# ANRGUSC/DEFER

Measured on NVIDIA H100. Metric: inferences_per_sec, higher is better.
Workload: dtype bf16x3->f32

## Files before the change

defer_b200/csrc/conv_umma.cu:

```cuda
#include <cuda.h>
#include <string.h>

#include <type_traits>

#include <vector>

#include "common.cuh"
#include "conv_umma.cuh"

namespace defer {

static int env_int(const char* name, int dflt) {
  const char* v = getenv(name);
  return v ? atoi(v) : dflt;
}

namespace {

constexpr int BM = 128;
constexpr int BK = 64;
constexpr int CONS_THREADS = 256;
constexpr int NUM_THREADS = CONS_THREADS + 128;
constexpr int SMEM_CAP = 227 * 1024 - 256;
constexpr int CTL_BYTES = 256;
// ... 7 lines not shown
  int tile_n, tile_h, tile_w, tiles_h, tiles_w;
  int flat;
  int m_total;
  int kh, kw, sh, sw, pad_t, pad_l;
  int cblocks;
  int k_blocks;
  int splits;
  int cluster;
  uint32_t flags;
  const float* scale;
  const float* shift;
  const void* res;
  void* y;
  float* partial;
  unsigned int* counters;
  size_t plane_out;
};

struct alignas(128) MegaOp {
  CUtensorMap tmx[2];
  CUtensorMap tmw[2];
  KParams p;
  int m_tiles, n_tiles;
  const float* stem_x;
  int stem_h, stem_w, stem_cin, stem_kh, stem_kw, stem_sh, stem_sw, stem_pad_t, stem_pad_l, stem_K;
  int stem_win_rows, stem_win_cols;
  const uint8_t* stem_u8;
  float stem_shift[3];
  const float* scale2;
  const float* shift2;
  void* y2;
  int relu2;
  int store_first;
};

template <int NPLANES, int BN>
struct Smem {
  static constexpr int A_PLANE = BM * 128;
  static constexpr int B_PLANE = BN * 128;
  static constexpr int STAGE = NPLANES * (A_PLANE + B_PLANE);
  static constexpr int RED = BM * BN * 4;
  __host__ __device__ static constexpr int ring(int stages, bool red) {
    return (red && stages * STAGE < RED) ? RED : stages * STAGE;
  }
  __host__ __device__ static constexpr int total(int stages, bool red) {
    return ring(stages, red) + STG_BYTES + CTL_BYTES + 1024;
  }
  __host__ __device__ static constexpr int max_stages() {
    return (SMEM_CAP - STG_BYTES - CTL_BYTES - 1024) / STAGE > MAX_STAGES ? MAX_STAGES
                                                                          : (SMEM_CAP - STG_BYTES - CTL_BYTES - 1024) / STAGE;
  }
};
static_assert(Smem<2, 128>::max_stages() == 3 && Smem<2, 64>::max_stages() == 4, "BF16X2 ring depths");
static_assert(Smem<1, 64>::max_stages() == 8 && Smem<1, 128>::max_stages() == 6, "BF16 ring depths");

__device__ __forceinline__ uint32_t smem_u32(const void* p) { return (uint32_t)__cvta_generic_to_shared(p); }

__device__ __forceinline__ void mbar_init(uint32_t bar, uint32_t count) {
  asm volatile("mbarrier.init.shared::cta.b64 [%0], %1;" ::"r"(bar), "r"(count));
}
__device__ __forceinline__ void mbar_arrive_expect_tx(uint32_t bar, uint32_t bytes) {
  asm volatile("mbarrier.arrive.expect_tx.shared::cta.b64 _, [%0], %1;" ::"r"(bar), "r"(bytes) : "memory");
}
__device__ __forceinline__ void mbar_expect_tx(uint32_t bar, uint32_t bytes) {
  asm volatile("mbarrier.expect_tx.relaxed.cta.shared::cta.b64 [%0], %1;" ::"r"(bar), "r"(bytes) : "memory");
}
// ... 147 lines not shown
  int cout;
  bool relu;
  bool store_first;
  bool relu2;
  const float* scale2;
  const float* shift2;
  __nv_bfloat16* y2;
};

__device__ __forceinline__ EpiArgs epi_args(const MegaOp& op) {
  const KParams& p = op.p;
  EpiArgs e;
  e.scale = p.scale;
  e.shift = p.shift;
  e.res = reinterpret_cast<const __nv_bfloat16*>(p.res);
  e.y = reinterpret_cast<__nv_bfloat16*>(p.y);
  e.plane = p.plane_out;
  e.cout = p.cout;
  e.relu = (p.flags & DEFER_FLAG_RELU) != 0;
  e.store_first = op.store_first != 0;
  e.relu2 = op.relu2 != 0;
  e.scale2 = op.scale2;
  e.shift2 = op.shift2;
  e.y2 = reinterpret_cast<__nv_bfloat16*>(op.y2);
  return e;
}

__device__ __forceinline__ uint32_t stg_off(int r, int c) {
  return (uint32_t)(r * STG_COLS + (((c >> 2) ^ ((r & 7) << 1)) << 2) + (c & 3)) * 4u;
}
__device__ __forceinline__ void sts2(uint32_t addr, float a, float b) {
  asm volatile("st.shared.v2.f32 [%0], {%1, %2};" ::"r"(addr), "f"(a), "f"(b));
}
__device__ __forceinline__ float4 lds4(uint32_t addr) {
  float4 v;
  asm volatile("ld.shared.v4.f32 {%0, %1, %2, %3}, [%4];" : "=f"(v.x), "=f"(v.y), "=f"(v.z), "=f"(v.w) : "r"(addr));
  return v;
}
__device__ __forceinline__ void stg4(void* p, uint4 v) {
  asm volatile("st.global.v4.b32 [%0], {%1, %2, %3, %4};" ::"l"(p), "r"(v.x), "r"(v.y), "r"(v.z), "r"(v.w));
}

__device__ __forceinline__ float bf_lo(uint32_t w) { return __uint_as_float(w << 16); }
__device__ __forceinline__ float bf_hi(uint32_t w) { return __uint_as_float(w & 0xffff0000u); }

template <int NPLANES, int BN, bool AFF>
__device__ __forceinline__ void epi_tile(const KParams& p, const EpiArgs& e, uint32_t stg, const float (&acc)[BN / 2],
                                         uint32_t qmask, int c_base, int n0, int h0, int w0) {
  const int tid = threadIdx.x;
  const int lane = tid & 31;
  const int row0 = (tid >> 7) * 64 + ((tid >> 5) & 3) * 16 + (lane >> 2);
  const int col_l = 2 * (lane & 3);
  const int jg = tid & 7;
  const int rb = tid >> 3;
  const int ca = 2 * jg + ((jg >> 2) & 1), cb = ca ^ 1;
  const bool swap = (jg >> 2) & 1;
  size_t orow[4];
  uint32_t vmask = 0;
#pragma unroll
  for (int k = 0; k < 4; ++k) {
    bool v;
    size_t pix;
    row_to_pixel(p, rb + 32 * k, n0, h0, w0, v, pix);
    orow[k] = pix * (size_t)e.cout;
    vmask |= (uint32_t)v << k;
  }
#pragma unroll
  for (int P = 0; P < BN / STG_COLS; ++P) {
    const bool mine = (qmask >> (8 * P + jg)) & 1u;
    const int c = c_base + STG_COLS * P + 8 * jg;
    cons_bar_sync();
#pragma unroll
    for (int qq = 0; qq < 8; ++qq) {
      const int q = 8 * P + qq;
      if (!((qmask >> q) & 1u)) continue;
      sts2(stg + stg_off(row0, 8 * qq + col_l), acc[4 * q], acc[4 * q + 1]);
      sts2(stg + stg_off(row0 + 8, 8 * qq + col_l), acc[4 * q + 2], acc[4 * q + 3]);
    }
    uint4 rh[4], rl[4];
// ... 20 lines not shown
        sf[0] = a.x; sf[1] = a.y; sf[2] = a.z; sf[3] = a.w; sf[4] = b.x; sf[5] = b.y; sf[6] = b.z; sf[7] = b.w;
      }
    }
    cons_bar_sync();
    if (!mine) continue;

#pragma unroll
    for (int k = 0; k < 4; ++k) {
      if (!((vmask >> k) & 1u)) continue;
      const int r = rb + 32 * k;
      const float4 xa = lds4(stg + stg_off(r, 4 * ca));
      const float4 xb = lds4(stg + stg_off(r, 4 * cb));
      const float4 x0 = swap ? xb : xa, x1 = swap ? xa : xb;
      float v[8] = {x0.x, x0.y, x0.z, x0.w, x1.x, x1.y, x1.z, x1.w};
      const uint32_t hw[4] = {rh[k].x, rh[k].y, rh[k].z, rh[k].w};
      const uint32_t lw[4] = {rl[k].x, rl[k].y, rl[k].z, rl[k].w};
#pragma unroll
      for (int i = 0; i < 8; ++i) {
        v[i] = fmaf(v[i], sc[i], sf[i]);
        if (e.res) {
          v[i] += (i & 1) ? bf_hi(hw[i >> 1]) : bf_lo(hw[i >> 1]);
          if (NPLANES == 2) v[i] += (i & 1) ? bf_hi(lw[i >> 1]) : bf_lo(lw[i >> 1]);
        }
        if (e.relu) v[i] = fmaxf(v[i], 0.f);
      }
      uint4 hi, lo = make_uint4(0u, 0u, 0u, 0u);
      if (NPLANES == 2) {
        split_bf16x2(v[0], v[1], hi.x, lo.x);
        split_bf16x2(v[2], v[3], hi.y, lo.y);
        split_bf16x2(v[4], v[5], hi.z, lo.z);
        split_bf16x2(v[6], v[7], hi.w, lo.w);
      } else {
        hi = make_uint4(pack_bf16x2(v[0], v[1]), pack_bf16x2(v[2], v[3]), pack_bf16x2(v[4], v[5]), pack_bf16x2(v[6], v[7]));
      }
      const size_t o = orow[k] + c;
      if (!AFF || e.store_first) {
        stg4(e.y + o, hi);
        if (NPLANES == 2) stg4(e.y + e.plane + o, lo);
      }
      if constexpr (AFF) {
        float s2[8], t2[8];
        {
          const float4 a = __ldg(reinterpret_cast<const float4*>(e.scale2 + c));
          const float4 b = __ldg(reinterpret_cast<const float4*>(e.scale2 + c + 4));
          const float4 d = __ldg(reinterpret_cast<const float4*>(e.shift2 + c));
          const float4 f = __ldg(reinterpret_cast<const float4*>(e.shift2 + c + 4));
          s2[0] = a.x; s2[1] = a.y; s2[2] = a.z; s2[3] = a.w; s2[4] = b.x; s2[5] = b.y; s2[6] = b.z; s2[7] = b.w;
          t2[0] = d.x; t2[1] = d.y; t2[2] = d.z; t2[3] = d.w; t2[4] = f.x; t2[5] = f.y; t2[6] = f.z; t2[7] = f.w;
        }
        const uint32_t sh[4] = {hi.x, hi.y, hi.z, hi.w};
        const uint32_t sl[4] = {lo.x, lo.y, lo.z, lo.w};
        float u[8];
#pragma unroll
        for (int i = 0; i < 8; ++i) {
          u[i] = (i & 1) ? bf_hi(sh[i >> 1]) : bf_lo(sh[i >> 1]);
          if (NPLANES == 2) u[i] = u[i] + ((i & 1) ? bf_hi(sl[i >> 1]) : bf_lo(sl[i >> 1]));
          u[i] = fmaf(u[i], s2[i], t2[i]);
          if (e.relu2) u[i] = fmaxf(u[i], 0.f);
        }
        uint4 h2, l2;
        if (NPLANES == 2) {
          split_bf16x2(u[0], u[1], h2.x, l2.x);
          split_bf16x2(u[2], u[3], h2.y, l2.y);
          split_bf16x2(u[4], u[5], h2.z, l2.z);
          split_bf16x2(u[6], u[7], h2.w, l2.w);
          stg4(e.y2 + o, h2);
// ... 337 lines not shown
template <int NPLANES>
__device__ __forceinline__ void stem_build(const StemGeo& g, uint32_t win, uint32_t a_dst, int r, int row_base, int kb) {
  int k = kb * BK;
  int a = k / g.run, jj = k - a * g.run;
  uint32_t src = win + 4u * (uint32_t)(row_base + a * g.wcols + jj);
  const uint32_t wrap = 4u * (uint32_t)(g.wcols - g.run);
#pragma unroll 1
  for (int ch = 0; ch < 8; ++ch) {
    float v[8];
#pragma unroll
    for (int e = 0; e < 8; ++e) {
      v[e] = 0.f;
      if (k < g.K) asm volatile("ld.shared.f32 %0, [%1];" : "=f"(v[e]) : "r"(src));
      ++k;
      src += 4u;
      if (++jj == g.run) { jj = 0; src += wrap; }
    }
    const uint32_t off = (uint32_t)r * 128u + ((uint32_t)(ch ^ (r & 7)) << 4);
    uint32_t h[4], l[4];
#pragma unroll
    for (int q = 0; q < 4; ++q) {
      if (NPLANES == 2) split_bf16x2(v[2 * q], v[2 * q + 1], h[q], l[q]);
      else h[q] = pack_bf16x2(v[2 * q], v[2 * q + 1]);
    }
    asm volatile("st.shared.v4.b32 [%0], {%1, %2, %3, %4};" ::"r"(a_dst + off), "r"(h[0]), "r"(h[1]), "r"(h[2]), "r"(h[3])
                 : "memory");
    if (NPLANES == 2)
      asm volatile("st.shared.v4.b32 [%0], {%1, %2, %3, %4};" ::"r"(a_dst + Smem<NPLANES, 64>::A_PLANE + off), "r"(l[0]),
                   "r"(l[1]), "r"(l[2]), "r"(l[3])
                   : "memory");
  }
}

template <int NPLANES, int IN>
__device__ __forceinline__ void stem_body(const MegaOp* ops, int stages, int pdl) {
  using L = Smem<NPLANES, 64>;
  extern __shared__ uint8_t smem_raw[];
  uint8_t* smem = reinterpret_cast<uint8_t*>((reinterpret_cast<uintptr_t>(smem_raw) + 1023) & ~(uintptr_t)1023);
  const uint32_t ring = smem_u32(smem);
  const uint32_t stg = ring + stages * L::STAGE;
  const uint32_t win0 = stg + STG_BYTES;
  const uint32_t bar_base = win0 + 2 * STEM_WIN_BYTES;
  auto full_bar = [&](int s) { return bar_base + 8u * s; };
  auto empty_bar = [&](int s) { return bar_base + 8u * (stages + s); };

  const int tid = threadIdx.x;
  if (tid == 0) {
    for (int s = 0; s < stages; ++s) {
      mbar_init(full_bar(s), 1);
      mbar_init(empty_bar(s), CONS_THREADS / 32);
    }
    asm volatile("fence.mbarrier_init.release.cluster;" ::: "memory");
  }
  __syncthreads();
  if (pdl) {
    asm volatile("griddepcontrol.wait;" ::: "memory");
    asm volatile("griddepcontrol.launch_dependents;" ::: "memory");
  }

  const MegaOp& op = ops[0];
  const KParams& p = op.p;
  const int total = op.m_tiles * op.n_tiles;
  const int k_blocks = p.k_blocks;
  uint32_t it = 0;

  if (tid >= CONS_THREADS) {
// ... 11 lines not shown
    }
    int wb = 0;
    for (int t = blockIdx.x; t < total; t += gridDim.x, wb ^= 1) {
      const int t_next = t + (int)gridDim.x;
      if (t_next < total) {
        stem_tile_origin(p, t_next % op.m_tiles, n0, h0, w0);
        stem_fill_load<IN>(g, ptid, n0, h0, w0, raw);
      }
      prod_bar_sync();
      const uint32_t win = win0 + (uint32_t)wb * STEM_WIN_BYTES;
      const int c_base = (t / op.m_tiles) * 64;
      for (int kb = 0; kb < k_blocks; ++kb, ++it) {
        const int stage = (int)(it % (uint32_t)stages);
        mbar_wait(empty_bar(stage), ((it / (uint32_t)stages) & 1u) ^ 1u, 1);
        const uint32_t a_dst = ring + stage * L::STAGE;
        const uint32_t b_dst = a_dst + NPLANES * L::A_PLANE;
        if (ptid == 0) {
          mbar_expect_tx(full_bar(stage), NPLANES * (uint32_t)L::B_PLANE);
          tma_load_3d(b_dst, &op.tmw[0], full_bar(stage), kb * BK, c_base, 0);
          if (NPLANES == 2) tma_load_3d(b_dst + L::B_PLANE, &op.tmw[1], full_bar(stage), kb * BK, c_base, 0);
        }
        stem_build<NPLANES>(g, win, a_dst, ptid, row_base, kb);
        asm volatile("fence.proxy.async.shared::cta;" ::: "memory");
        prod_bar_sync();
        if (ptid == 0) mbar_arrive(full_bar(stage));
      }
      if (t_next < total) stem_fill_store<IN>(g, win0 + (uint32_t)(wb ^ 1) * STEM_WIN_BYTES, ptid, raw);
    }
    return;
  }

  const int wg = tid >> 7;
  const int lane = tid & 31;
  for (int t = blockIdx.x; t < total; t += gridDim.x) {
    float acc[32];
#pragma unroll
    for (int i = 0; i < 32; ++i) acc[i] = 0.f;
    int prev_stage = -1;
    for (int kb = 0; kb < k_blocks; ++kb, ++it) {
      const int stage = (int)(it % (uint32_t)stages);
      mbar_wait(full_bar(stage), (it / (uint32_t)stages) & 1u, 2);
      const uint32_t a_addr = ring + stage * L::STAGE + wg * (64 * 128);
      const uint32_t b_addr = ring + stage * L::STAGE + NPLANES * L::A_PLANE;
      wg_fence();
#pragma unroll
      for (int k = 0; k < BK / 16; ++k) {
        const uint64_t a_hi = make_sw128_desc(a_addr + k * 32);
        const uint64_t b_hi = make_sw128_desc(b_addr + k * 32);
        wgmma_bf16<64>(acc, a_hi, b_hi);
        if (NPLANES == 2) {
          wgmma_bf16<64>(acc, make_sw128_desc(a_addr + L::A_PLANE + k * 32), b_hi);
          wgmma_bf16<64>(acc, a_hi, make_sw128_desc(b_addr + L::B_PLANE + k * 32));
        }
      }
      wg_commit();
      wg_wait<1>();
      acc_fence(acc);
      if (prev_stage >= 0 && lane == 0) mbar_arrive(empty_bar(prev_stage));
      prev_stage = stage;
    }
    wg_wait<0>();
    acc_fence(acc);
    if (prev_stage >= 0 && lane == 0) mbar_arrive(empty_bar(prev_stage));
    int n0, h0, w0;
    stem_tile_origin(p, t % op.m_tiles, n0, h0, w0);
    epi_tile<NPLANES, 64, false>(p, epi_args(op), stg, acc, 0xffffu, (t / op.m_tiles) * 64, n0, h0, w0);
  }
}

template <int NPLANES>
__global__ void __launch_bounds__(NUM_THREADS, 1) conv_stem_kernel(const MegaOp* __restrict__ ops, int stages, int pdl) {
  stem_body<NPLANES, STEM_F32>(ops, stages, pdl);
}

template <int NPLANES>
__global__ void __launch_bounds__(NUM_THREADS, 1) conv_stem_u8_kernel(const MegaOp* __restrict__ ops, int stages, int pdl) {
  stem_body<NPLANES, STEM_U8_CAFFE>(ops, stages, pdl);
}

template <int NPLANES>
__global__ void __launch_bounds__(NUM_THREADS, 1) conv_stem_u8tf_kernel(const MegaOp* __restrict__ ops, int stages, int pdl) {
  stem_body<NPLANES, STEM_U8_TF>(ops, stages, pdl);
}

__global__ void __launch_bounds__(256) weight_transform_kernel(const float* __restrict__ w, __nv_bfloat16* __restrict__ out,
                                                               int taps, int cin, int cout, int nplanes) {
  size_t total = (size_t)taps * cin * cout;
  size_t i = (size_t)blockIdx.x * blockDim.x + threadIdx.x;
  if (i >= total) return;
  int ci = (int)(i % cin);
  size_t t2 = i / cin;
  int co = (int)(t2 % cout);
  int tap = (int)(t2 / cout);
  float v = w[((size_t)tap * cin + ci) * cout + co];
  __nv_bfloat16 hi = __float2bfloat16_rn(v);
  out[i] = hi;
  if (nplanes == 2) out[total + i] = __float2bfloat16_rn(v - __bfloat162float(hi));
}

// ... 441 lines not shown
bool umma_stem_fusable(int fmt, int cin, int ho, int wo, int cout, int kh, int kw, int sh, int sw, uint32_t flags) {
  if (fmt != FMT_BF16X2 && fmt != FMT_BF16) return false;
  if (cout != 64 || (flags & DEFER_FLAG_RESIDUAL) || kh * kw * cin > 256) return false;
  int tile_h, tile_w, win_rows, win_cols;
  stem_tile(ho, wo, kh, kw, sh, sw, cin, &tile_h, &tile_w, &win_rows, &win_cols);
  return (long long)win_rows * win_cols <= STEM_WIN_VALS;
}

int umma_mega_set_stem(void* host_op, const float* x, int h, int w, int cin, int kh, int kw, int sh, int sw, int pad_t,
                       int pad_l) {
  MegaOp* op = reinterpret_cast<MegaOp*>(host_op);
  KParams& p = op->p;
  op->stem_x = x;
  op->stem_h = h; op->stem_w = w; op->stem_cin = cin;
  op->stem_kh = kh; op->stem_kw = kw; op->stem_sh = sh; op->stem_sw = sw;
  op->stem_pad_t = pad_t; op->stem_pad_l = pad_l;
  op->stem_K = kh * kw * cin;
  stem_tile(p.ho, p.wo, kh, kw, sh, sw, cin, &p.tile_h, &p.tile_w, &op->stem_win_rows, &op->stem_win_cols);
  p.flat = 0;
  p.tile_n = 1;
  p.tiles_h = (p.ho + p.tile_h - 1) / p.tile_h;
  p.tiles_w = (p.wo + p.tile_w - 1) / p.tile_w;
  op->m_tiles = p.n * p.tiles_h * p.tiles_w;
  return op->m_tiles * op->n_tiles;
}

void umma_mega_set_stem_u8(void* host_op, const uint8_t* x, const float shift[3]) {
  MegaOp* op = reinterpret_cast<MegaOp*>(host_op);
  op->stem_x = nullptr;
  op->stem_u8 = x;
  for (int c = 0; c < 3; ++c) op->stem_shift[c] = shift[c];
}

int launch_conv_stem(int nplanes, const void* dev_op, int n_tiles, bool u8, bool tf, cudaStream_t st) {
  const int stages = env_int("DEFER_STREAM_STAGES", MAX_STAGES);
  if (u8 && tf)
    return nplanes == 2 ? launch_stem_t<2, STEM_U8_TF>(dev_op, n_tiles, stages, st)
                        : launch_stem_t<1, STEM_U8_TF>(dev_op, n_tiles, stages, st);
  if (u8)
    return nplanes == 2 ? launch_stem_t<2, STEM_U8_CAFFE>(dev_op, n_tiles, stages, st)
                        : launch_stem_t<1, STEM_U8_CAFFE>(dev_op, n_tiles, stages, st);
  return nplanes == 2 ? launch_stem_t<2, STEM_F32>(dev_op, n_tiles, stages, st) : launch_stem_t<1, STEM_F32>(dev_op, n_tiles, stages, st);
}

int launch_conv_mega(int nplanes, const void* dev_ops, int n_ops, cudaStream_t st) {
  int stages = env_int("DEFER_MEGA_STAGES", 4);
  return nplanes == 2 ? launch_mega_t<2>(dev_ops, n_ops, stages, st) : launch_mega_t<1>(dev_ops, n_ops, stages, st);
}

void umma_conv_release(UmmaConvPlan& P) {
  if (P.w_dev) cudaFree(P.w_dev);
  P.w_dev = nullptr;
  P.ready = false;
}

}
```

defer_b200/csrc/conv_umma.cuh:

```cuda
#pragma once
#include <cuda.h>
#include <cuda_runtime.h>
#include <stdint.h>

namespace defer {

struct UmmaConvPlan {
  int fmt = 0, nplanes = 1;
  int n = 0, h = 0, w = 0, cin = 0, ho = 0, wo = 0, cout = 0;
  int kh = 1, kw = 1, sh = 1, sw = 1, pad_t = 0, pad_l = 0;
  uint32_t flags = 0;
  int tile_n = 1, tile_h = 1, tile_w = 1, tiles_n = 1, tiles_h = 1, tiles_w = 1;
  int flat = 0;
  int bn = 64;
  int k_blocks = 0;
  int splits = 1;
  int cluster = 0;
  int stages = 4;
  int stream = 0;
  void* w_dev = nullptr;
  const float* scale = nullptr;
  const float* shift = nullptr;
  bool aff = false;
  const float* scale2 = nullptr;
// ... 2 lines not shown
  int store_first = 1;
  CUtensorMap tmap_w[2];
  bool ready = false;
};

struct UmmaConvLaneArgs {
  CUtensorMap tmap_x[2];
  bool direct_out = false;
  const void* res = nullptr;
  void* y = nullptr;
  void* y2 = nullptr;
  float* partial = nullptr;
  unsigned int* counters = nullptr;
};

bool umma_conv_supported(int fmt, int n, int h, int w, int cin, int ho, int wo, int cout, int kh, int kw, int sh, int sw,
                         int pad_t, int pad_l);
int umma_conv_prepare(UmmaConvPlan* plan, int fmt, int n, int h, int w, int cin, int ho, int wo, int cout, int kh, int kw,
                      int sh, int sw, int pad_t, int pad_l, uint32_t flags, const float* w_hwio_dev, const float* scale_dev,
                      const float* shift_dev, bool mega = false, int stream_bn = 0);
int umma_conv_bind(const UmmaConvPlan& plan, UmmaConvLaneArgs* args, const void* x, const void* res, void* y);
void umma_conv_unbind(UmmaConvLaneArgs* args);
int launch_conv_umma(const UmmaConvPlan& plan, const UmmaConvLaneArgs& args, cudaStream_t st);
void umma_conv_release(UmmaConvPlan& plan);

size_t umma_mega_op_bytes();
int umma_mega_fill(void* host_dst, const UmmaConvPlan& plan, const UmmaConvLaneArgs& args);
int umma_mega_cluster_size();
int launch_conv_mega(int nplanes, const void* dev_ops, int n_ops, cudaStream_t st);
int launch_conv_stream(int nplanes, int bn, const void* dev_op, int n_tiles, int k_blocks, bool aff, cudaStream_t st);
bool umma_stem_fusable(int fmt, int cin, int ho, int wo, int cout, int kh, int kw, int sh, int sw, uint32_t flags);
int umma_mega_set_stem(void* host_op, const float* x, int h, int w, int cin, int kh, int kw, int sh, int sw, int pad_t, int pad_l);
void umma_mega_set_stem_u8(void* host_op, const uint8_t* x, const float shift[3]);
int launch_conv_stem(int nplanes, const void* dev_op, int n_tiles, bool u8, bool tf, cudaStream_t st);
int launch_conv_persistent(int nplanes, const void* dev_op, int n_tiles, bool aff, cudaStream_t st);

}
```

defer_b200/csrc/stage.cu:

```cuda
#include <stdarg.h>
#include <string.h>
#include <unistd.h>

#include <mutex>
#include <set>
#include <utility>
#include <stdlib.h>
#include <string>
#include <vector>

#include "common.cuh"
#include "conv_umma.cuh"

namespace defer {

static thread_local char g_err[1024] = "";
void set_error(const char* fmt, ...) {
  va_list ap;
  va_start(ap, fmt);
  vsnprintf(g_err, sizeof(g_err), fmt, ap);
  va_end(ap);
}
const char* get_error() { return g_err; }

void prefer_max_smem_impl(const void* func) {
  static std::mutex mu;
  static std::set<std::pair<const void*, int>> done;
  int dev = 0;
  if (cudaGetDevice(&dev) != cudaSuccess) return;
  std::lock_guard<std::mutex> lk(mu);
  if (done.count({func, dev})) return;
  if (getenv("DEFER_NO_CARVEOUT") == nullptr)
    cudaFuncSetAttribute(func, cudaFuncAttributePreferredSharedMemoryCarveout, cudaSharedmemCarveoutMaxShared);
  cudaGetLastError();
  done.insert({func, dev});
}
// ... 17 lines not shown
  uint64_t off_slots;
  uint64_t slot_stride;
  uint64_t local_base;
  cudaIpcMemHandle_t ipc;
};
static_assert(sizeof(LinkToken) <= DEFER_LINK_TOKEN_BYTES, "token too large");
constexpr uint32_t TOKEN_MAGIC = 0xDEFE7B20u;

struct Buf {
  int h, w, c, elem;
  size_t elems;
  size_t bytes;
};

struct OpRt {
  defer_op_desc d;
  int backend = 1;
  int k_pad = 0;
  void* w_pad = nullptr;
  bool persist = false;
  bool stem_fused = false;
  bool stream = false;
  int n_tiles64 = 0;
  int stem_tiles = 0;
  UmmaConvPlan umma;
  std::string kname;
  double alg_bytes = 0, alg_flops = 0;
  int n_kernels = 1;
  float pre_shift[3] = {0.f, 0.f, 0.f};
  int folded_into = -1;
  int u8_pre = -1;
  int aff_op = -1;
  bool store_out = true;
};

struct Lane {
  cudaStream_t stream = nullptr;
  std::vector<void*> buf;
  cudaGraphExec_t exec = nullptr;
  cudaGraph_t graph = nullptr;
  cudaEvent_t done = nullptr, t0 = nullptr, t1 = nullptr, join = nullptr;
  float* out_host = nullptr;
  int* status_host = nullptr;
  float* dense_partial = nullptr;
  std::vector<UmmaConvLaneArgs> umma;
  std::vector<void*> persist_op;
  std::vector<void*> im2col;
  bool timed = false;
  void* peer_out = nullptr;
  int32_t* tables = nullptr;
  bool stepped = false;
  uint64_t last_seq = 0;
};

enum HopMode { HOP_COPY = 0, HOP_TMA = 1, HOP_DIRECT = 2 };

struct Mark {
  cudaEvent_t ev = nullptr;
  bool recorded = false;
};

}

using namespace defer;

struct defer_stage_s {
  defer_stage_config cfg;
  std::vector<Buf> bufs;
  std::vector<OpRt> ops;
  std::vector<void*> d_weights;
  std::vector<size_t> weight_bytes;
  std::vector<void*> d_weights_bf16;
  std::vector<Lane> lanes;
  uint8_t* arena = nullptr;
  size_t arena_bytes = 0, slot_stride = 0;
  std::vector<void*> workspace;
  bool has_prod = false, has_cons = false, finalized = false, unlinked = false;
  uint8_t* cons_arena = nullptr;
  size_t cons_off_slots = 0, cons_slot_stride = 0;
  uint8_t* prod_arena = nullptr;
// ... 46 lines not shown
  const int fmt = s->cfg.fmt, nb = s->cfg.batch;
  const Buf& bi = s->bufs[d.in0];
  const Buf& bo = s->bufs[d.out];
  void* x = L.buf[d.in0];
  void* y = L.buf[d.out];
  auto wptr = [&](int id) -> const float* { return id >= 0 ? (const float*)s->d_weights[id] : nullptr; };
  switch (d.kind) {
    case DEFER_OP_CONV: {
      if (op.backend == 4 && op.stem_fused)
        return launch_conv_stem(op.umma.nplanes, L.persist_op[oi], op.stem_tiles, op.u8_pre >= 0,
                                op.u8_pre >= 0 && s->ops[op.u8_pre].d.mode == DEFER_PRE_TF, st);
      if (op.backend == 4)
        DEFER_TRY(launch_stem_im2col(fmt, (const float*)x, L.im2col[oi], nb, bi.h, bi.w, bi.c, d.kh, d.kw, d.sh, d.sw, d.pad_t,
                                     d.pad_l, bo.h, bo.w, op.k_pad, st));
      if (op.backend == 2 || op.backend == 4) {
        if (op.stream)
          return launch_conv_stream(op.umma.nplanes, op.umma.bn, L.persist_op[oi],
                                    op.umma.tiles_n * op.umma.tiles_h * op.umma.tiles_w * (op.umma.cout / op.umma.bn),
                                    op.umma.k_blocks, op.aff_op >= 0, st);
        if (op.persist) return launch_conv_persistent(op.umma.nplanes, L.persist_op[oi], op.n_tiles64, op.aff_op >= 0, st);
        return launch_conv_umma(op.umma, L.umma[oi], st);
      }
      ConvParams p;
      p.x = x; p.w = wptr(d.w_kernel); p.scale = wptr(d.w_scale); p.shift = wptr(d.w_shift);
      p.res = (d.flags & DEFER_FLAG_RESIDUAL) ? L.buf[d.in1] : nullptr;
      p.y = y;
      p.n = nb; p.h = bi.h; p.w_in = bi.w; p.cin = bi.c;
      p.ho = bo.h; p.wo = bo.w; p.cout = bo.c;
      p.kh = d.kh; p.kw = d.kw; p.sh = d.sh; p.sw = d.sw; p.pad_t = d.pad_t; p.pad_l = d.pad_l;
      p.flags = d.flags;
      return launch_conv_simt(fmt, bi.elem == DEFER_BUF_F32, p, st);
    }
    case DEFER_OP_MAXPOOL:
      return launch_maxpool(fmt, x, y, nb, bi.h, bi.w, bi.c, d.kh, d.kw, d.sh, d.sw, d.pad_t, d.pad_l, bo.h, bo.w, st);
    case DEFER_OP_GAP:
      return launch_gap(fmt, x, y, nb, bi.h, bi.w, bi.c, st);
    case DEFER_OP_DENSE: {
      int F = bi.h * bi.w * bi.c, U = bo.c;
      bool wb = s->d_weights_bf16[d.w_kernel] != nullptr;
      const void* w = wb ? s->d_weights_bf16[d.w_kernel] : s->d_weights[d.w_kernel];
      return launch_dense(fmt, x, w, wb, wptr(d.w_shift), y, bo.elem == DEFER_BUF_F32, L.dense_partial, nb, F, U,
                          d.flags, st);
    }
    case DEFER_OP_SOFTMAX:
      return launch_softmax((const float*)x, (float*)y, nb, bo.c, st);
    case DEFER_OP_AFFINE:
      if (op.folded_into >= 0) return DEFER_OK;
      [[fallthrough]];
    case DEFER_OP_RELU:
    case DEFER_OP_ADD:
      return launch_eltwise(fmt, d.kind, x, d.in1 >= 0 ? L.buf[d.in1] : nullptr, wptr(d.w_scale), wptr(d.w_shift), y,
                            (size_t)nb * bi.h * bi.w, bi.c, d.flags, st);
    case DEFER_OP_PAD:
      return launch_pad(fmt, x, y, nb, bi.h, bi.w, bi.c, d.pad_t, d.pad_l, bo.h, bo.w, st);
    case DEFER_OP_COPY:
      if (bi.elem == bo.elem) {
        if (bi.elem == DEFER_BUF_F32) {
          DEFER_CUDA(cudaMemcpyAsync(y, x, bi.elems * 4, cudaMemcpyDeviceToDevice, st));
          return DEFER_OK;
        }
        return launch_copy_act(fmt, x, y, bi.elems, st);
      }
      if (bi.elem == DEFER_BUF_F32) return launch_encode(fmt, (const float*)x, y, bi.elems, st);
      return launch_decode(fmt, x, (float*)y, bi.elems, st);
    case DEFER_OP_PREPROCESS:
      if (op.folded_into >= 0) return DEFER_OK;
// ... 842 lines not shown
        if (L.im2col.size() < s->ops.size()) L.im2col.resize(s->ops.size(), nullptr);
        if (!L.im2col[oi] && !op.stem_fused) {
          const size_t bytes = (size_t)s->cfg.batch * bo.h * bo.w * op.k_pad * fmt_bytes_per_elem(s->cfg.fmt);
          DEFER_CUDA(cudaMalloc(&L.im2col[oi], bytes));
          s->workspace.push_back(L.im2col[oi]);
        }
        conv_in = op.stem_fused ? L.buf[d.out] : L.im2col[oi];
      }
      DEFER_TRY(umma_conv_bind(op.umma, &L.umma[oi], conv_in,
                               (d.flags & DEFER_FLAG_RESIDUAL) ? L.buf[d.in1] : nullptr, L.buf[d.out]));
      if (op.aff_op >= 0) L.umma[oi].y2 = L.buf[s->ops[op.aff_op].d.out];
    }
  }
  for (int pi = 0; pi < (int)s->ops.size(); ++pi) {
    OpRt& pre = s->ops[pi];
    if (pre.d.kind != DEFER_OP_PREPROCESS || pre.d.out == s->cfg.output_buf) continue;
    int reader = -1, n_reads = 0;
    for (int oi = 0; oi < (int)s->ops.size(); ++oi) {
      const defer_op_desc& d = s->ops[oi].d;
      const int r = (d.in0 == pre.d.out) + (d.in1 == pre.d.out);
      if (r) reader = oi;
      n_reads += r;
    }
    if (n_reads != 1 || s->ops[reader].d.kind != DEFER_OP_CONV || !s->ops[reader].stem_fused) continue;
    OpRt& conv = s->ops[reader];
    pre.folded_into = reader;
    pre.n_kernels = 0;
    pre.alg_bytes = 0;
    conv.u8_pre = pi;
    conv.kname = pre.d.mode == DEFER_PRE_TF ? "conv_stem_u8tf_kernel" : "conv_stem_u8_kernel";
    pre.kname = "preprocess (fused into " + conv.kname + ")";
    conv.alg_bytes -= (double)s->bufs[pre.d.in0].elems * 3.0;
  }
  for (int oi = 0; oi < (int)s->ops.size(); ++oi) {
    OpRt& op = s->ops[oi];
    if ((op.backend != 2 && op.backend != 4) || !op.persist) continue;
    const size_t ob = umma_mega_op_bytes();
    std::vector<uint8_t> host(ob);
    for (int l = 0; l < s->cfg.depth; ++l) {
      Lane& L = s->lanes[l];
      L.persist_op.resize(s->ops.size(), nullptr);
      DEFER_TRY(umma_mega_fill(host.data(), op.umma, L.umma[oi]));
      if (op.stem_fused) {
        const defer_op_desc& d = op.d;
        const Buf& bi = s->bufs[d.in0];
        op.stem_tiles = umma_mega_set_stem(host.data(), (const float*)L.buf[d.in0], bi.h, bi.w, bi.c, d.kh, d.kw, d.sh, d.sw,
                                           d.pad_t, d.pad_l);
        if (op.u8_pre >= 0) {
          const OpRt& pre = s->ops[op.u8_pre];
          umma_mega_set_stem_u8(host.data(), (const uint8_t*)L.buf[pre.d.in0], pre.pre_shift);
        }
      }
      DEFER_CUDA(cudaMalloc(&L.persist_op[oi], ob));
      s->workspace.push_back(L.persist_op[oi]);
      DEFER_CUDA(cudaMemcpy(L.persist_op[oi], host.data(), ob, cudaMemcpyHostToDevice));
    }
  }
  for (auto& g : s->groups) {
    const int n = g.last - g.first + 1;
    const size_t ob = umma_mega_op_bytes();
    std::vector<uint8_t> host(ob * n);
    g.dev_ops.assign(s->cfg.depth, nullptr);
    for (int l = 0; l < s->cfg.depth; ++l) {
      for (int k = 0; k < n; ++k)
        DEFER_TRY(umma_mega_fill(host.data() + ob * k, s->ops[g.first + k].umma, s->lanes[l].umma[g.first + k]));
      DEFER_CUDA(cudaMalloc(&g.dev_ops[l], ob * n));
      s->workspace.push_back(g.dev_ops[l]);
      DEFER_CUDA(cudaMemcpy(g.dev_ops[l], host.data(), ob * n, cudaMemcpyHostToDevice));
    }
  }
  DEFER_CUDA(cudaDeviceSynchronize());
  if (s->cfg.use_graph) {
    for (int l = 0; l < s->cfg.depth; ++l) {
      Lane& L = s->lanes[l];
      DEFER_CUDA(cudaStreamBeginCapture(L.stream, cudaStreamCaptureModeThreadLocal));
      int rc = enqueue_lane(s, l, L.stream);
      cudaError_t e = cudaStreamEndCapture(L.stream, &L.graph);
      if (rc != DEFER_OK) return rc;
      DEFER_CUDA(e);
      DEFER_CUDA(cudaGraphInstantiate(&L.exec, L.graph, 0));
    }
  }
  s->finalized = true;
  return DEFER_OK;
// ... 201 lines not shown
  Mark& m = s->marks[slot];
  if (!m.ev) DEFER_CUDA(cudaEventCreate(&m.ev));
  DEFER_CUDA(cudaEventRecord(m.ev, s->lanes[seq % s->cfg.depth].stream));
  m.recorded = true;
  return DEFER_OK;
}

int defer_stage_mark_elapsed(defer_stage_t s, float* ms) {
  DEFER_CHECK(s && ms, "mark_elapsed: null");
  DEFER_CHECK(s->marks[0].recorded && s->marks[1].recorded, "mark_elapsed: both marks must have been recorded");
  DEFER_TRY(set_device(s));
  DEFER_CUDA(cudaEventSynchronize(s->marks[0].ev));
  DEFER_CUDA(cudaEventSynchronize(s->marks[1].ev));
  DEFER_CUDA(cudaEventElapsedTime(ms, s->marks[0].ev, s->marks[1].ev));
  return DEFER_OK;
}

int defer_stage_num_kernels(defer_stage_t s, int* per_step) {
  DEFER_CHECK(s && per_step, "num_kernels: null");
  int n = 0;
  for (size_t i = 0; i < s->ops.size(); ++i) {
    auto& op = s->ops[i];
    const int g = s->op_group.empty() ? -1 : s->op_group[i];
    if (g >= 0 && (int)i != s->groups[g].first) continue;
    bool is_memcpy = op.d.kind == DEFER_OP_COPY && s->bufs[op.d.in0].elem == DEFER_BUF_F32 && s->bufs[op.d.out].elem == DEFER_BUF_F32;
    if (!is_memcpy) n += op.n_kernels;
  }
  if (s->has_prod) n += 2;
  if (s->has_cons) n += 2;
  *per_step = n;
  return DEFER_OK;
}

int defer_stage_read_buffer(defer_stage_t s, int lane, int buf_id, float* host_out, uint64_t n_floats) {
  DEFER_CHECK(s && host_out && lane >= 0 && lane < s->cfg.depth && buf_id >= 0 && buf_id < (int)s->bufs.size(),
              "read_buffer: bad arguments");
  const Buf& b = s->bufs[buf_id];
  DEFER_CHECK(n_floats == b.elems, "read_buffer: buffer has %zu elements, caller asked %llu", b.elems,
              (unsigned long long)n_floats);
  DEFER_TRY(set_device(s));
  void* src = s->lanes[lane].buf[buf_id];
  DEFER_CHECK(src, "read_buffer: buffer %d is not bound yet", buf_id);
  for (size_t i = 0; i < s->ops.size(); ++i) {
    const OpRt& op = s->ops[i];
    if (op.d.out != buf_id) continue;
    DEFER_CHECK(!(op.d.kind == DEFER_OP_PREPROCESS && op.folded_into >= 0),
                "read_buffer: buffer %d is never written: op %zu (preprocess) is folded into op %d (%s)", buf_id, i,
                op.folded_into, op.folded_into >= 0 ? s->ops[op.folded_into].kname.c_str() : "");
    DEFER_CHECK(op.store_out, "read_buffer: buffer %d is never written: op %zu (%s) stores only the output of the affine op %d "
                "folded into it (no other op reads buffer %d; without DEFER_FOLD_AFFINE=1 it is written)", buf_id, i, op.kname.c_str(),
                op.aff_op, buf_id);
  }
  DEFER_CUDA(cudaStreamSynchronize(s->lanes[lane].stream));
  if (b.elem == DEFER_BUF_U8) {
    std::vector<uint8_t> raw(b.elems);
    DEFER_CUDA(cudaMemcpy(raw.data(), src, b.elems, cudaMemcpyDeviceToHost));
    for (size_t i = 0; i < b.elems; ++i) host_out[i] = (float)raw[i];
    return DEFER_OK;
  }
  if (b.elem == DEFER_BUF_F32 || s->cfg.fmt == DEFER_FMT_F32) {
    DEFER_CUDA(cudaMemcpy(host_out, src, b.elems * 4, cudaMemcpyDeviceToHost));
    return DEFER_OK;
  }
  float* tmp = nullptr;
  DEFER_CUDA(cudaMalloc((void**)&tmp, b.elems * 4));
  int rc = launch_decode(s->cfg.fmt, src, tmp, b.elems, 0);
  cudaError_t e = cudaMemcpy(host_out, tmp, b.elems * 4, cudaMemcpyDeviceToHost);
  cudaFree(tmp);
  if (rc != DEFER_OK) return rc;
  DEFER_CUDA(e);
  return DEFER_OK;
}

int defer_stage_stream(defer_stage_t s, int lane, void** stream) {
  DEFER_CHECK(s && stream && lane >= 0 && lane < s->cfg.depth, "stream: bad arguments");
  *stream = (void*)s->lanes[lane].stream;
  return DEFER_OK;
}

int defer_stage_time_op(defer_stage_t s, int op_index, int iters, int flush_l2, float* us_per_launch) {
  DEFER_CHECK(s && us_per_launch && op_index >= 0 && op_index < (int)s->ops.size() && iters >= 1, "time_op: bad arguments");
  DEFER_CHECK(s->finalized, "time_op: finalize first");
  DEFER_TRY(set_device(s));
  Lane& L = s->lanes[0];
  const defer_op_desc& d = s->ops[op_index].d;
  DEFER_CHECK(L.buf[d.out] && L.buf[d.in0], "time_op: op buffers not bound");
  DEFER_CHECK(s->ops[op_index].folded_into < 0, "time_op: op %d launches nothing, it is folded into op %d (%s)", op_index,
              s->ops[op_index].folded_into, s->ops[op_index].folded_into >= 0 ? s->ops[s->ops[op_index].folded_into].kname.c_str() : "");
  if (flush_l2 && !s->flush_buf) {
    s->flush_bytes = 256ull << 20;
    DEFER_CUDA(cudaMalloc(&s->flush_buf, s->flush_bytes));
  }
  DEFER_CUDA(cudaStreamSynchronize(L.stream));
  for (int i = 0; i < 3; ++i) DEFER_TRY(launch_op(s, 0, op_index, L.stream));
  double total_ms = 0;
  if (flush_l2) {
    for (int i = 0; i < iters; ++i) {
      DEFER_CUDA(cudaMemsetAsync(s->flush_buf, i & 0xff, s->flush_bytes, L.stream));
      DEFER_CUDA(cudaEventRecord(L.t0, L.stream));
      DEFER_TRY(launch_op(s, 0, op_index, L.stream));
      DEFER_CUDA(cudaEventRecord(L.t1, L.stream));
      DEFER_CUDA(cudaEventSynchronize(L.t1));
      float ms = 0;
      DEFER_CUDA(cudaEventElapsedTime(&ms, L.t0, L.t1));
      total_ms += ms;
    }
  } else {
    DEFER_CUDA(cudaEventRecord(L.t0, L.stream));
    for (int i = 0; i < iters; ++i) DEFER_TRY(launch_op(s, 0, op_index, L.stream));
    DEFER_CUDA(cudaEventRecord(L.t1, L.stream));
    DEFER_CUDA(cudaEventSynchronize(L.t1));
    float ms = 0;
    DEFER_CUDA(cudaEventElapsedTime(&ms, L.t0, L.t1));
    total_ms = ms;
  }
  *us_per_launch = (float)(total_ms * 1000.0 / iters);
  return DEFER_OK;
}

int defer_stage_op_info(defer_stage_t s, int op_index, double* alg_bytes, double* alg_flops, char* kernel_name,
                        int name_len) {
// ... 32 lines not shown
```

Baseline: 14280.

## Fold 3x3 stride-2 maxpool into the stem conv epilogue with border partials

When the stem conv's output is read only by a 3x3/s2/p1 maxpool, the conv epilogue now stages the decoded tile in shared memory and computes the interior pooled outputs directly. Windows that cross tile borders write per-tile partial maxima to a workspace, and a small border kernel merges them. This removes the full-resolution stem activation write and the separate maxpool read. In exchange it adds partial-buffer traffic, an extra launch, and re-running the stem conv whenever the stem output buffer is read back.

```diff
diff --git a/defer_b200/csrc/conv_umma.cu b/defer_b200/csrc/conv_umma.cu
--- a/defer_b200/csrc/conv_umma.cu
+++ b/defer_b200/csrc/conv_umma.cu
@@ -63,6 +63,8 @@
   void* y2;
   int relu2;
   int store_first;
+  void* pool_y;
+  float* pool_part;
 };
 
 template <int NPLANES, int BN>
@@ -276,6 +278,9 @@
 __device__ __forceinline__ void sts2(uint32_t addr, float a, float b) {
   asm volatile("st.shared.v2.f32 [%0], {%1, %2};" ::"r"(addr), "f"(a), "f"(b));
 }
+__device__ __forceinline__ void sts4(uint32_t addr, float4 v) {
+  asm volatile("st.shared.v4.f32 [%0], {%1, %2, %3, %4};" ::"r"(addr), "f"(v.x), "f"(v.y), "f"(v.z), "f"(v.w));
+}
 __device__ __forceinline__ float4 lds4(uint32_t addr) {
   float4 v;
   asm volatile("ld.shared.v4.f32 {%0, %1, %2, %3}, [%4];" : "=f"(v.x), "=f"(v.y), "=f"(v.z), "=f"(v.w) : "r"(addr));
@@ -288,7 +293,7 @@
 __device__ __forceinline__ float bf_lo(uint32_t w) { return __uint_as_float(w << 16); }
 __device__ __forceinline__ float bf_hi(uint32_t w) { return __uint_as_float(w & 0xffff0000u); }
 
-template <int NPLANES, int BN, bool AFF>
+template <int NPLANES, int BN, bool AFF, bool DECODE = false>
 __device__ __forceinline__ void epi_tile(const KParams& p, const EpiArgs& e, uint32_t stg, const float (&acc)[BN / 2],
                                          uint32_t qmask, int c_base, int n0, int h0, int w0) {
   const int tid = threadIdx.x;
@@ -375,6 +380,19 @@
         split_bf16x2(v[6], v[7], hi.w, lo.w);
       } else {
         hi = make_uint4(pack_bf16x2(v[0], v[1]), pack_bf16x2(v[2], v[3]), pack_bf16x2(v[4], v[5]), pack_bf16x2(v[6], v[7]));
+      }
+      if constexpr (DECODE) {
+        const uint32_t sh[4] = {hi.x, hi.y, hi.z, hi.w};
+        const uint32_t sl[4] = {lo.x, lo.y, lo.z, lo.w};
+        float u[8];
+#pragma unroll
+        for (int i = 0; i < 8; ++i) {
+          u[i] = (i & 1) ? bf_hi(sh[i >> 1]) : bf_lo(sh[i >> 1]);
+          if (NPLANES == 2) u[i] = u[i] + ((i & 1) ? bf_hi(sl[i >> 1]) : bf_lo(sl[i >> 1]));
+        }
+        sts4(stg + stg_off(r, 8 * jg), make_float4(u[0], u[1], u[2], u[3]));
+        sts4(stg + stg_off(r, 8 * jg + 4), make_float4(u[4], u[5], u[6], u[7]));
+        continue;
       }
       const size_t o = orow[k] + c;
       if (!AFF || e.store_first) {
@@ -778,6 +796,115 @@
   }
 }
 
+constexpr int POOL_SLOTS = 24;
+constexpr int POOL_TILE_H = 8;
+static_assert(POOL_TILE_H * STEM_TILE_W == BM, "a stem tile is 8 x 16 conv pixels");
+
+__device__ __forceinline__ void pool_window(uint32_t stg, int jg, int r0, int r1, int c0, int c1, float (&m)[8]) {
+  for (int r = r0; r <= r1; ++r)
+    for (int c = c0; c <= c1; ++c) {
+      const int row = r * STEM_TILE_W + c;
+      const float4 x = lds4(stg + stg_off(row, 8 * jg)), y = lds4(stg + stg_off(row, 8 * jg + 4));
+      m[0] = fmaxf(m[0], x.x); m[1] = fmaxf(m[1], x.y); m[2] = fmaxf(m[2], x.z); m[3] = fmaxf(m[3], x.w);
+      m[4] = fmaxf(m[4], y.x); m[5] = fmaxf(m[5], y.y); m[6] = fmaxf(m[6], y.z); m[7] = fmaxf(m[7], y.w);
+    }
+}
+
+template <int NPLANES>
+__device__ __forceinline__ void pool_store(__nv_bfloat16* y, size_t plane, size_t o, const float (&m)[8]) {
+  uint4 hi, lo;
+  if (NPLANES == 2) {
+    split_bf16x2(m[0], m[1], hi.x, lo.x);
+    split_bf16x2(m[2], m[3], hi.y, lo.y);
+    split_bf16x2(m[4], m[5], hi.z, lo.z);
+    split_bf16x2(m[6], m[7], hi.w, lo.w);
+    stg4(y + o, hi);
+    stg4(y + plane + o, lo);
+  } else {
+    hi = make_uint4(pack_bf16x2(m[0], m[1]), pack_bf16x2(m[2], m[3]), pack_bf16x2(m[4], m[5]), pack_bf16x2(m[6], m[7]));
+    stg4(y + o, hi);
+  }
+}
+
+__device__ __forceinline__ void pool_part_store(float* slot, int jg, const float (&m)[8]) {
+  __stcg(reinterpret_cast<float4*>(slot + 8 * jg), make_float4(m[0], m[1], m[2], m[3]));
+  __stcg(reinterpret_cast<float4*>(slot + 8 * jg + 4), make_float4(m[4], m[5], m[6], m[7]));
+}
+__device__ __forceinline__ void pool_part_max(const float* slot, int jg, float (&m)[8]) {
+  const float4 x = __ldcg(reinterpret_cast<const float4*>(slot + 8 * jg));
+  const float4 y = __ldcg(reinterpret_cast<const float4*>(slot + 8 * jg + 4));
+  m[0] = fmaxf(m[0], x.x); m[1] = fmaxf(m[1], x.y); m[2] = fmaxf(m[2], x.z); m[3] = fmaxf(m[3], x.w);
+  m[4] = fmaxf(m[4], y.x); m[5] = fmaxf(m[5], y.y); m[6] = fmaxf(m[6], y.z); m[7] = fmaxf(m[7], y.w);
+}
+
+template <int NPLANES>
+__device__ __forceinline__ void stem_pool_tile(const MegaOp& op, uint32_t stg, int m_tile) {
+  const KParams& p = op.p;
+  const int tid = threadIdx.x;
+  const int jg = tid & 7;
+  const int t2 = m_tile / p.tiles_w;
+  const int n = t2 / p.tiles_h, a = t2 - n * p.tiles_h, b = m_tile - t2 * p.tiles_w;
+  const int pho = p.ho / 2, pwo = p.wo / 2;
+  auto part = [&](int tile, int slot) { return op.pool_part + ((size_t)tile * POOL_SLOTS + slot) * 64; };
+  cons_bar_sync();
+  {
+    const int q = tid >> 3, i = q >> 3, j = q & 7;
+    float m[8];
+#pragma unroll
+    for (int e = 0; e < 8; ++e) m[e] = -INFINITY;
+    pool_window(stg, jg, i == 0 ? 0 : 2 * i - 1, 2 * i + 1, j == 0 ? 0 : 2 * j - 1, 2 * j + 1, m);
+    if (i > 0 && j > 0)
+      pool_store<NPLANES>(reinterpret_cast<__nv_bfloat16*>(op.pool_y), (size_t)p.n * pho * pwo * 64,
+                          (((size_t)n * pho + 4 * a + i) * pwo + 8 * b + j) * 64 + 8 * jg, m);
+    else
+      pool_part_store(part(m_tile, i == 0 ? j : 7 + i), jg, m);
+  }
+  if (tid < 13 * 8) {
+    const int q = tid >> 3;
+    const bool down = a + 1 < p.tiles_h, right = b + 1 < p.tiles_w;
+    float m[8];
+#pragma unroll
+    for (int e = 0; e < 8; ++e) m[e] = -INFINITY;
+    if (q < 8 && down) {
+      pool_window(stg, jg, 7, 7, q == 0 ? 0 : 2 * q - 1, 2 * q + 1, m);
+      pool_part_store(part(m_tile + p.tiles_w, 11 + q), jg, m);
+    } else if (q >= 8 && q < 12 && right) {
+      const int i = q - 8;
+      pool_window(stg, jg, i == 0 ? 0 : 2 * i - 1, 2 * i + 1, 15, 15, m);
+      pool_part_store(part(m_tile + 1, 19 + i), jg, m);
+    } else if (q == 12 && down && right) {
+      pool_window(stg, jg, 7, 7, 15, 15, m);
+      pool_part_store(part(m_tile + p.tiles_w + 1, 23), jg, m);
+    }
+  }
+}
+
+template <int NPLANES>
+__global__ void __launch_bounds__(256) stem_pool_border_kernel(const float* __restrict__ part, __nv_bfloat16* __restrict__ y,
+                                                               int n, int tiles_h, int tiles_w) {
+  const int m_tiles = n * tiles_h * tiles_w;
+  const int idx = blockIdx.x * blockDim.x + threadIdx.x;
+  if (idx >= m_tiles * 11 * 8) return;
+  const int jg = idx & 7, bp = (idx >> 3) % 11, tile = (idx >> 3) / 11;
+  const int t2 = tile / tiles_w;
+  const int nn = t2 / tiles_h, a = t2 - nn * tiles_h, b = tile - t2 * tiles_w;
+  const int i = bp < 8 ? 0 : bp - 7, j = bp < 8 ? bp : 0;
+  const float* slots = part + (size_t)tile * POOL_SLOTS * 64;
+  float m[8];
+#pragma unroll
+  for (int e = 0; e < 8; ++e) m[e] = -INFINITY;
+  pool_part_max(slots + bp * 64, jg, m);
+  if (i == 0 && a > 0) pool_part_max(slots + (11 + j) * 64, jg, m);
+  if (j == 0 && b > 0) pool_part_max(slots + (19 + i) * 64, jg, m);
+  if (i == 0 && j == 0 && a > 0 && b > 0) pool_part_max(slots + 23 * 64, jg, m);
+  if ((i == 0 && a == 0) || (j == 0 && b == 0)) {
+#pragma unroll
+    for (int e = 0; e < 8; ++e) m[e] = fmaxf(m[e], 0.f);
+  }
+  const int pho = tiles_h * 4, pwo = tiles_w * 8;
+  pool_store<NPLANES>(y, (size_t)n * pho * pwo * 64, (((size_t)nn * pho + 4 * a + i) * pwo + 8 * b + j) * 64 + 8 * jg, m);
+}
+
 template <int NPLANES, int IN>
 __device__ __forceinline__ void stem_body(const MegaOp* ops, int stages, int pdl) {
   using L = Smem<NPLANES, 64>;
@@ -855,6 +982,7 @@
 
   const int wg = tid >> 7;
   const int lane = tid & 31;
+  const bool pool = op.pool_y != nullptr;
   for (int t = blockIdx.x; t < total; t += gridDim.x) {
     float acc[32];
 #pragma unroll
@@ -887,7 +1015,12 @@
     if (prev_stage >= 0 && lane == 0) mbar_arrive(empty_bar(prev_stage));
     int n0, h0, w0;
     stem_tile_origin(p, t % op.m_tiles, n0, h0, w0);
-    epi_tile<NPLANES, 64, false>(p, epi_args(op), stg, acc, 0xffffu, (t / op.m_tiles) * 64, n0, h0, w0);
+    if (pool) {
+      epi_tile<NPLANES, 64, false, true>(p, epi_args(op), stg, acc, 0xffffu, 0, n0, h0, w0);
+      stem_pool_tile<NPLANES>(op, stg, t);
+    } else {
+      epi_tile<NPLANES, 64, false>(p, epi_args(op), stg, acc, 0xffffu, (t / op.m_tiles) * 64, n0, h0, w0);
+    }
   }
 }
 
@@ -1395,6 +1528,36 @@
   for (int c = 0; c < 3; ++c) op->stem_shift[c] = shift[c];
 }
 
+bool umma_stem_pool_foldable(int ho, int wo, uint32_t stem_flags, int ph, int pw, int sh, int sw, int pad_t, int pad_l,
+                             int pho, int pwo) {
+  return (stem_flags & DEFER_FLAG_RELU) && ph == 3 && pw == 3 && sh == 2 && sw == 2 && pad_t == 1 && pad_l == 1 &&
+         ho % POOL_TILE_H == 0 && wo % STEM_TILE_W == 0 && pho == ho / 2 && pwo == wo / 2;
+}
+
+size_t umma_stem_pool_part_bytes(int m_tiles) { return (size_t)m_tiles * POOL_SLOTS * 64 * sizeof(float); }
+
+void umma_mega_set_stem_pool(void* host_op, void* y, void* pool_y, float* part) {
+  MegaOp* op = reinterpret_cast<MegaOp*>(host_op);
+  op->p.y = y;
+  op->pool_y = pool_y;
+  op->pool_part = part;
+}
+
+int launch_stem_pool_border(int nplanes, const float* part, void* y, int n, int ho, int wo, cudaStream_t st) {
+  const int tiles_h = ho / POOL_TILE_H, tiles_w = wo / STEM_TILE_W;
+  const unsigned grid = (unsigned)(((size_t)n * tiles_h * tiles_w * 11 * 8 + 255) / 256);
+  __nv_bfloat16* yb = reinterpret_cast<__nv_bfloat16*>(y);
+  if (nplanes == 2) {
+    prefer_max_smem(stem_pool_border_kernel<2>);
+    stem_pool_border_kernel<2><<<grid, 256, 0, st>>>(part, yb, n, tiles_h, tiles_w);
+  } else {
+    prefer_max_smem(stem_pool_border_kernel<1>);
+    stem_pool_border_kernel<1><<<grid, 256, 0, st>>>(part, yb, n, tiles_h, tiles_w);
+  }
+  DEFER_CUDA(cudaGetLastError());
+  return DEFER_OK;
+}
+
 int launch_conv_stem(int nplanes, const void* dev_op, int n_tiles, bool u8, bool tf, cudaStream_t st) {
   const int stages = env_int("DEFER_STREAM_STAGES", MAX_STAGES);
   if (u8 && tf)
diff --git a/defer_b200/csrc/conv_umma.cuh b/defer_b200/csrc/conv_umma.cuh
--- a/defer_b200/csrc/conv_umma.cuh
+++ b/defer_b200/csrc/conv_umma.cuh
@@ -58,6 +58,11 @@
 bool umma_stem_fusable(int fmt, int cin, int ho, int wo, int cout, int kh, int kw, int sh, int sw, uint32_t flags);
 int umma_mega_set_stem(void* host_op, const float* x, int h, int w, int cin, int kh, int kw, int sh, int sw, int pad_t, int pad_l);
 void umma_mega_set_stem_u8(void* host_op, const uint8_t* x, const float shift[3]);
+bool umma_stem_pool_foldable(int ho, int wo, uint32_t stem_flags, int ph, int pw, int sh, int sw, int pad_t, int pad_l,
+                             int pho, int pwo);
+size_t umma_stem_pool_part_bytes(int m_tiles);
+void umma_mega_set_stem_pool(void* host_op, void* y, void* pool_y, float* part);
+int launch_stem_pool_border(int nplanes, const float* part, void* y, int n, int ho, int wo, cudaStream_t st);
 int launch_conv_stem(int nplanes, const void* dev_op, int n_tiles, bool u8, bool tf, cudaStream_t st);
 int launch_conv_persistent(int nplanes, const void* dev_op, int n_tiles, bool aff, cudaStream_t st);
 
diff --git a/defer_b200/csrc/stage.cu b/defer_b200/csrc/stage.cu
--- a/defer_b200/csrc/stage.cu
+++ b/defer_b200/csrc/stage.cu
@@ -2,6 +2,7 @@
 #include <string.h>
 #include <unistd.h>
 
+#include <algorithm>
 #include <mutex>
 #include <set>
 #include <utility>
@@ -85,6 +86,7 @@
   int u8_pre = -1;
   int aff_op = -1;
   bool store_out = true;
+  int pool_op = -1;
 };
 
 struct Lane {
@@ -99,6 +101,7 @@
   std::vector<UmmaConvLaneArgs> umma;
   std::vector<void*> persist_op;
   std::vector<void*> im2col;
+  float* pool_part = nullptr;
   bool timed = false;
   void* peer_out = nullptr;
   int32_t* tables = nullptr;
@@ -211,6 +214,8 @@
       return launch_conv_simt(fmt, bi.elem == DEFER_BUF_F32, p, st);
     }
     case DEFER_OP_MAXPOOL:
+      if (op.folded_into >= 0)
+        return launch_stem_pool_border(s->ops[op.folded_into].umma.nplanes, L.pool_part, y, nb, bi.h, bi.w, st);
       return launch_maxpool(fmt, x, y, nb, bi.h, bi.w, bi.c, d.kh, d.kw, d.sh, d.sw, d.pad_t, d.pad_l, bo.h, bo.w, st);
     case DEFER_OP_GAP:
       return launch_gap(fmt, x, y, nb, bi.h, bi.w, bi.c, st);
@@ -1119,6 +1124,42 @@
     pre.kname = "preprocess (fused into " + conv.kname + ")";
     conv.alg_bytes -= (double)s->bufs[pre.d.in0].elems * 3.0;
   }
+  for (int ci = 0; ci < (int)s->ops.size(); ++ci) {
+    OpRt& conv = s->ops[ci];
+    if (!conv.stem_fused || conv.d.out == s->cfg.output_buf) continue;
+    int reader = -1, n_reads = 0;
+    for (int oi = 0; oi < (int)s->ops.size(); ++oi) {
+      const defer_op_desc& d = s->ops[oi].d;
+      const int r = (d.in0 == conv.d.out) + (d.in1 == conv.d.out);
+      if (r) reader = oi;
+      n_reads += r;
+    }
+    if (n_reads != 1 || s->ops[reader].d.kind != DEFER_OP_MAXPOOL) continue;
+    OpRt& pool = s->ops[reader];
+    const defer_op_desc& pd = pool.d;
+    const Buf& bc = s->bufs[conv.d.out];
+    const Buf& bp = s->bufs[pd.out];
+    if (!umma_stem_pool_foldable(bc.h, bc.w, conv.d.flags, pd.kh, pd.kw, pd.sh, pd.sw, pd.pad_t, pd.pad_l, bp.h, bp.w)) continue;
+    const int m_tiles = s->cfg.batch * (bc.h / 8) * (bc.w / 16);
+    const double part_b = (double)umma_stem_pool_part_bytes(m_tiles);
+    pool.folded_into = ci;
+    conv.pool_op = reader;
+    pool.kname = "stem_pool_border_kernel";
+    conv.alg_bytes += bp.bytes * 21.0 / 32.0 + part_b - (double)bc.bytes;
+    pool.alg_bytes = part_b + bp.bytes * 11.0 / 32.0;
+    if (s->output_writer == reader) s->output_writer = ci;
+    for (int l = 0; l < s->cfg.depth; ++l) {
+      Lane& L = s->lanes[l];
+      if (!L.pool_part) {
+        DEFER_CUDA(cudaMalloc((void**)&L.pool_part, umma_stem_pool_part_bytes(m_tiles)));
+        s->workspace.push_back(L.pool_part);
+      }
+      void*& out = L.buf[conv.d.out];
+      s->workspace.erase(std::find(s->workspace.begin(), s->workspace.end(), out));
+      DEFER_CUDA(cudaFree(out));
+      out = nullptr;
+    }
+  }
   for (int oi = 0; oi < (int)s->ops.size(); ++oi) {
     OpRt& op = s->ops[oi];
     if ((op.backend != 2 && op.backend != 4) || !op.persist) continue;
@@ -1137,6 +1178,8 @@
           const OpRt& pre = s->ops[op.u8_pre];
           umma_mega_set_stem_u8(host.data(), (const uint8_t*)L.buf[pre.d.in0], pre.pre_shift);
         }
+        if (op.pool_op >= 0)
+          umma_mega_set_stem_pool(host.data(), nullptr, L.buf[s->ops[op.pool_op].d.out], L.pool_part);
       }
       DEFER_CUDA(cudaMalloc(&L.persist_op[oi], ob));
       s->workspace.push_back(L.persist_op[oi]);
@@ -1404,6 +1447,32 @@
   return DEFER_OK;
 }
 
+static int recompute_stem_out(defer_stage_t s, int lane, int oi) {
+  Lane& L = s->lanes[lane];
+  const OpRt& op = s->ops[oi];
+  void*& out = L.buf[op.d.out];
+  if (!out) {
+    DEFER_CUDA(cudaMalloc(&out, (s->bufs[op.d.out].bytes + 255) / 256 * 256));
+    s->workspace.push_back(out);
+  }
+  const size_t ob = umma_mega_op_bytes();
+  std::vector<uint8_t> host(ob);
+  DEFER_CUDA(cudaMemcpy(host.data(), L.persist_op[oi], ob, cudaMemcpyDeviceToHost));
+  umma_mega_set_stem_pool(host.data(), out, nullptr, nullptr);
+  void* dev_op = nullptr;
+  DEFER_CUDA(cudaMalloc(&dev_op, ob));
+  int rc = cudaMemcpy(dev_op, host.data(), ob, cudaMemcpyHostToDevice) == cudaSuccess ? DEFER_OK : DEFER_ERR_CUDA;
+  if (rc == DEFER_OK)
+    rc = launch_conv_stem(op.umma.nplanes, dev_op, op.stem_tiles, op.u8_pre >= 0,
+                          op.u8_pre >= 0 && s->ops[op.u8_pre].d.mode == DEFER_PRE_TF, L.stream);
+  if (cudaStreamSynchronize(L.stream) != cudaSuccess && rc == DEFER_OK) {
+    set_error("read_buffer: recomputing the stem output failed: %s", cudaGetErrorString(cudaGetLastError()));
+    rc = DEFER_ERR_CUDA;
+  }
+  cudaFree(dev_op);
+  return rc;
+}
+
 int defer_stage_read_buffer(defer_stage_t s, int lane, int buf_id, float* host_out, uint64_t n_floats) {
   DEFER_CHECK(s && host_out && lane >= 0 && lane < s->cfg.depth && buf_id >= 0 && buf_id < (int)s->bufs.size(),
               "read_buffer: bad arguments");
@@ -1411,6 +1480,8 @@
   DEFER_CHECK(n_floats == b.elems, "read_buffer: buffer has %zu elements, caller asked %llu", b.elems,
               (unsigned long long)n_floats);
   DEFER_TRY(set_device(s));
+  for (size_t i = 0; i < s->ops.size(); ++i)
+    if (s->ops[i].d.out == buf_id && s->ops[i].pool_op >= 0) DEFER_TRY(recompute_stem_out(s, lane, (int)i));
   void* src = s->lanes[lane].buf[buf_id];
   DEFER_CHECK(src, "read_buffer: buffer %d is not bound yet", buf_id);
   for (size_t i = 0; i < s->ops.size(); ++i) {
@@ -1455,10 +1526,12 @@
   DEFER_CHECK(s->finalized, "time_op: finalize first");
   DEFER_TRY(set_device(s));
   Lane& L = s->lanes[0];
-  const defer_op_desc& d = s->ops[op_index].d;
-  DEFER_CHECK(L.buf[d.out] && L.buf[d.in0], "time_op: op buffers not bound");
-  DEFER_CHECK(s->ops[op_index].folded_into < 0, "time_op: op %d launches nothing, it is folded into op %d (%s)", op_index,
-              s->ops[op_index].folded_into, s->ops[op_index].folded_into >= 0 ? s->ops[s->ops[op_index].folded_into].kname.c_str() : "");
+  const OpRt& op = s->ops[op_index];
+  const bool pooled = op.d.kind == DEFER_OP_MAXPOOL && op.folded_into >= 0;
+  DEFER_CHECK(op.folded_into < 0 || pooled, "time_op: op %d launches nothing, it is folded into op %d (%s)", op_index, op.folded_into,
+              op.folded_into >= 0 ? s->ops[op.folded_into].kname.c_str() : "");
+  const int out = op.pool_op >= 0 ? s->ops[op.pool_op].d.out : op.d.out;
+  DEFER_CHECK(L.buf[out] && (pooled ? (const void*)L.pool_part : L.buf[op.d.in0]), "time_op: op buffers not bound");
   if (flush_l2 && !s->flush_buf) {
     s->flush_bytes = 256ull << 20;
     DEFER_CUDA(cudaMalloc(&s->flush_buf, s->flush_bytes));
```

Result: faster. 14470 (median of 6 runs) (+1.3%).
